# jyakaranda/A-LeGO-LOAM

Measured on AMD Instinct MI355X. Metric: scans/sec (16x1800 LiDAR) full IP->LO->LM loop, higher is better.
Workload: dtype f32/f64

## Files before the change

a-lego-loam_amd/csrc/alego_api.hip:

```cpp
#include <hip/hip_runtime.h>

#include <cmath>
#include <cstdio>
#include <cstdlib>
#include <algorithm>
#include <cstring>
#include <mutex>
#include <string>
#include <vector>

#include "../../include/alego_mi355x.h"
#include "api_gate.h"
#include "dev_common.h"
#include "dev_mem.h"
#include "front_end.h"
#include "lm_ctx.h"
#include "lm_host.h"
#include "merge_math.h"
#include "nn_rules.h"
#include "thin_math.h"
#include "occ_math.h"
#include "loop_ctx.h"
#include "pgraph.h"
#include "prof.h"
// ... 1778 lines not shown
    *count = (int)bytes; *dtype = 3;
    return 0;
  }
  if (s.rfind("rl_", 0) == 0) {
    if (s == "rl_stats") {
      if (cap_bytes < 8) { h->err = "debug_get: buffer too small"; return ALEGO_ERR_CAPACITY; }
      reloc_debug_stats(h->rl, (int*)out);
      *count = 2; *dtype = 2;
      return 0;
    }
    const void* rsrc = nullptr;
    size_t bytes = 0;
    if (reloc_debug_get(h->rl, slot, name, &rsrc, &bytes)) { h->err = std::string("debug_get: ") + name + " needs alego_reloc_enable"; return ALEGO_ERR_ARG; }
    if ((size_t)cap_bytes < bytes) { h->err = "debug_get: buffer too small"; return ALEGO_ERR_CAPACITY; }
    if (bytes) HIP_TRY(h, hipMemcpy(out, rsrc, bytes, hipMemcpyDeviceToHost));
    *count = (int)bytes; *dtype = 3;
    return 0;
  }
  if (s == "fe_cand_span") {
    if (cap_bytes < 8) { h->err = "debug_get: buffer too small"; return ALEGO_ERR_CAPACITY; }
    ((int*)out)[0] = fe_cand_span(d); ((int*)out)[1] = fe_sector_cap(d);
    *count = 2; *dtype = 2;
    return 0;
  }
  if (s == "fe_cand_counts" || s == "fe_cand_lists") {
    if (!fe_fused_eligible(d)) { h->err = "debug_get: " + s + " needs the fused feature extraction"; return ALEGO_ERR_ARG; }
    const bool lists = s == "fe_cand_lists";
    const size_t row = lists ? (size_t)d.P.n_sectors * fe_sector_cap(d) * sizeof(uint2) : (size_t)d.P.n_sectors * 2 * sizeof(int);
    const void* src = lists ? (const void*)st_cand_of(d, slot, 0) : (const void*)st_idx_of(d, slot, 0, F_LFLAT);
    const size_t pitch = lists ? (size_t)((const char*)st_cand_of(d, slot, 1) - (const char*)st_cand_of(d, slot, 0)) : (size_t)((const char*)st_idx_of(d, slot, 1, F_LFLAT) - (const char*)st_idx_of(d, slot, 0, F_LFLAT));
    if ((size_t)cap_bytes < row * d.NS) { h->err = "debug_get: buffer too small"; return ALEGO_ERR_CAPACITY; }
    HIP_TRY(h, hipMemcpy2D(out, row, src, pitch, row, d.NS, hipMemcpyDeviceToHost));
    *count = (int)(row * d.NS / 4); *dtype = 2;
    return 0;
  }
  const size_t base = (size_t)slot * d.N, M = sc[SC_M];
  const size_t fb = fbuf(slot, sc[SC_CUR]);
  int fc[F_KINDS];
  HIP_TRY(h, hipMemcpy(fc, feat_cnt_of(d, fb), sizeof(fc), hipMemcpyDeviceToHost));
  static const char* const cloud[F_KINDS] = {"sharp", "less_sharp", "flat", "less_flat"};
  struct Row { std::string name; const void* row; size_t n; int dtype; };
  std::vector<Row> tab = {
    {"range_img", d.range_img + base, (size_t)d.N, 0}, {"label_img", d.label_img + base, (size_t)d.N, 2}, {"flag_img", d.flag_img + base, (size_t)d.N, 3},
    {"owner", d.owner + base, (size_t)d.N, 2}, {"parent", d.parent + base, (size_t)d.N, 2},
    {"seg_cloud", d.seg_pts + base, M * 4, 0}, {"outlier", d.outlier + base, (size_t)sc[SC_NOUT] * 4, 0},
    {"imu_ptr", imu_ptr_of(d, slot), IMP_N, 2}, {"imu_ring", imu_ring_of(d, slot), imu_ring_n(), 1},
    {"seg_ground", d.seg_ground + base, M, 3}, {"seg_col", d.seg_col + base, M, 2}, {"seg_range", d.seg_range + base, M, 0},
    {"ring_start", ring_start_of(d, slot, 0), (size_t)d.NS, 2}, {"ring_end", ring_end_of(d, slot, 0), (size_t)d.NS, 2},
    {"orientation", ori_of(d, slot), ORI_N, 0}, {"scal", scal_of(d, slot), SC_COUNT, 2},
    {"curv_d", d.cd + base, M, 0}, {"picked_occl", d.picked0 + base, M, 3}, {"point_label", d.plabel + base, M, 2},
    {"lo_surf_corr", lo_corr_of(d, slot, 0), (size_t)fc[F_FLAT] * LC_W, 2}, {"lo_corner_corr", lo_corr_of(d, slot, 1), (size_t)fc[F_SHARP] * LC_W, 2},
    {"lo_state", lo_state_of(d, slot), LO_STATE_N, 1}, {"poses", poses_of(d, slot), PO_W, 1}};
  if (d.P.deskew_mode) tab.push_back({"undistorted", d.seg_dsk + base, (size_t)sc[SC_M_DSK] * 4, 0});
  for (int k = 0; k < F_KINDS; ++k) {
    tab.push_back({cloud[k], feat_of(d, k, fb), (size_t)fc[k] * 4, 0});
    if (k < F_LFLAT) tab.push_back({std::string(cloud[k]) + "_idx", feat_idx_of(d, k, fb), (size_t)fc[k], 2});
  }
  const Row* hit = nullptr;
  for (const Row& r : tab) if (r.name == s) hit = &r;
  if (!hit) return lm_host_debug_get(h->lm, slot, name, out, cap_bytes, count, dtype, &h->err);
  const void* src = hit->row;
  const size_t n = hit->n, esz = hit->dtype == 1 ? 8 : hit->dtype == 3 ? 1 : 4;
  const int dt = hit->dtype;
  if ((size_t)cap_bytes < n * esz) { h->err = "debug_get: buffer too small"; return ALEGO_ERR_CAPACITY; }
  if (n) HIP_TRY(h, hipMemcpy(out, src, n * esz, hipMemcpyDeviceToHost));
  *count = (int)n; *dtype = dt;
  return 0;
}

}
```

a-lego-loam_amd/csrc/kernels_fe2.hip:

```cpp
#include <algorithm>
#include <cstdlib>
#include "dev_common.h"
#include "fe_common.h"
#include "front_end.h"
#include "prof.h"
#include "vgrid.h"

#define FE_MAXH 4096

#ifndef FF_G
#define FF_G 4
#endif
#define FF_LPR (64 / FF_G)
#define FF_HALO 8
#ifndef FC_SPAN
#define FC_SPAN 0
#endif
#ifndef FC_NW
#define FC_NW 4
#endif
#define FF_WIN 256

struct FfLayout {
  int cols, wave_bytes;
// ... 281 lines not shown
    const int ns = R.act0 ? cc[2 * j] : 0, nf = R.act0 ? cc[2 * j + 1] : 0;
    uint2* lst = ff_list(d, slot, rc, j, sector_cap);
    for (int w = gl; w < mw; w += FF_LPR) mk[w] = 0u;
    const int nsw = (int)wave_max_u32((uint32_t)ns), nfw = (int)wave_max_u32((uint32_t)nf);
    constexpr int KU = 32 / FF_LPR;
    if (nsw <= (BIG ? 64 : 32)) ff_pick_regs<(BIG ? 2 : 1) * KU, false>(P, R, ns, lst, 1, mk, mw, gl);
    else if (nsw <= (BIG ? 128 : 64)) ff_pick_regs<(BIG ? 4 : 2) * KU, false>(P, R, ns, lst, 1, mk, mw, gl);
    else if (nsw <= (BIG ? 192 : 96) && !d.opt_fe_cand) ff_pick_regs<(BIG ? 6 : 3) * KU, false>(P, R, ns, lst, 1, mk, mw, gl);
    else ff_pick_mem<false>(P, R, ns, nsw, lst, 1, mk, mw, gl);
    __builtin_amdgcn_wave_barrier();
    if (nfw <= 32 && !(d.opt_fe_cand && nfw > 8)) ff_pick_regs<KU, true>(P, R, nf, lst + sector_cap - 1, -1, mk, mw, gl);
    else if (BIG && nfw <= 64 && !d.opt_fe_cand) ff_pick_regs<2 * KU, true>(P, R, nf, lst + sector_cap - 1, -1, mk, mw, gl);
    else ff_pick_mem<true>(P, R, nf, nfw, lst + sector_cap - 1, -1, mk, mw, gl);
    __builtin_amdgcn_wave_barrier();
  }
  if (rv && gl == 0) {
    int* c = st_cnt_of(d, slot, ring);
    c[F_SHARP] = R.n_sharp; c[F_LSHARP] = R.n_ls; c[F_FLAT] = R.n_flat;
  }
}

#ifndef FO_BLOCK
#define FO_BLOCK 256
#endif
#define FO_NB 256
#define FO_U 4
#define FO_CAP_PCT 72
#define FO_INVALID 0xFFFFFFFFu
#define FO_END 0xFFFFu
#define FO_SPIN_LIMIT (1 << 22)
#define FO_ALIAS_INTS (6 * ((FE_MAXH + LO_CH - 1) / LO_CH) > 768 ? 6 * ((FE_MAXH + LO_CH - 1) / LO_CH) : 768)
#define FO_STATIC_LDS (928 + 4 * FO_ALIAS_INTS)
#ifndef FO_BUDGET_BIG
#define FO_BUDGET_BIG 53248
#endif
#ifndef FO_KEYED
#define FO_KEYED 1
#endif
#ifndef FO_STAGE
#define FO_STAGE 0
#endif
struct FoLayout { int cap; int keyed; };
__host__ __device__ inline FoLayout fo_layout(int H) {
  const int budget = 12 * H + FO_STATIC_LDS > 40960 ? FO_BUDGET_BIG : 40960;
  FoLayout L;
  L.keyed = FO_KEYED && 14 * H + FO_STATIC_LDS <= budget;
  const int by_pct = (H * FO_CAP_PCT / 100 + 15) & ~15, by_lds = (budget - FO_STATIC_LDS - (L.keyed ? 14 : 12) * H) / 16;
  L.cap = !FO_STAGE || by_lds <= 0 ? 0 : (by_pct < by_lds ? by_pct : (by_lds & ~15));
  return L;
}
static size_t fo_lds_bytes(int H) { const FoLayout L = fo_layout(H); return std::max((size_t)(L.keyed ? 14 : 12) * H + (size_t)16 * L.cap, (size_t)6 * 65 * 4); }

DEV_INLINE uint32_t mad_u24(uint32_t a, uint32_t b, uint32_t c) { uint32_t r; asm("v_mad_u32_u24 %0, %1, %2, %3" : "=v"(r) : "v"(a), "v"(b), "v"(c)); return r; }

#ifdef ALEGO_TIMING
__device__ long long fo_times[24];
extern "C" void alego_fo_times(long long* out) { (void)hipMemcpyFromSymbol(out, HIP_SYMBOL(fo_times), sizeof(long long) * 24); }
#ifndef FO_TICK_RING
#define FO_TICK_RING 8
#endif
#define FO_TICK(k) do { if (threadIdx.x == 0 && ring == FO_TICK_RING && blockIdx.x == 0) fo_times[k] = wall_clock64(); } while (0)
#elif defined(FO_STOP_AFTER)
#define FO_TICK(k) do { if ((k) == FO_STOP_AFTER) { if (threadIdx.x == 0) __hip_atomic_store(fe_sync_of(d, slot, ring), (epoch << 16), __ATOMIC_RELAXED, __HIP_MEMORY_SCOPE_AGENT); return; } } while (0)
#else
#define FO_TICK(k)
#endif

DEV_INLINE void fo_picks_out(const DevCtx& d, int slot, unsigned char* smem) {
  fe_concat_picks<FO_BLOCK>(d, slot, fbuf(slot, cur_in_flight(d, slot)), reinterpret_cast<int (*)[65]>(smem), d.n_launch == 1);
}

__global__ void __launch_bounds__(FO_BLOCK) fe_ring_out(DevCtx d) {
  const int slot = blockIdx.x + d.slot0, tid = threadIdx.x, lane = tid & 63;
  const int NS = d.NS, H = d.H;
  extern __shared__ __attribute__((aligned(16))) unsigned char fo_smem[];
  if ((int)blockIdx.x >= d.n_launch) return;
  if ((int)blockIdx.y == NS) { fo_picks_out(d, slot, fo_smem); return; }
  int* scv = scal_of(d, slot);
  __shared__ int s_ticket;
  if (tid == 0) s_ticket = atomicAdd(&scv[SC_FE_TICKET], 1);
  __syncthreads();
  const int ring = min(s_ticket, NS - 1);
  const size_t base = (size_t)slot * d.N;
  const alego_params& P = d.P;
  const int cur = cur_in_flight(d, slot);
  const size_t fb = fbuf(slot, cur);
  const unsigned epoch = (unsigned)scv[SC_FE_EPOCH] & 0xFFFFu;
  const int S = *ring_start_of(d, slot, ring), E = *ring_end_of(d, slot, ring);
  const int n_all = min(max(E - S, 0), H);
  const int n_ls = st_cnt_of(d, slot, ring)[F_LSHARP];
  const int* st_ls = st_idx_of(d, slot, ring, F_LSHARP);
  const float4* seg = d.seg_lo + base;
  float4* s_pt = reinterpret_cast<float4*>(fo_smem);
  const FoLayout lay = fo_layout(H);
  const int cap = lay.cap;
  unsigned char* fv2 = fo_smem + (size_t)16 * cap;
  uint32_t* s_key = reinterpret_cast<uint32_t*>(fv2);
  uint16_t* s_tmp = reinterpret_cast<uint16_t*>(fv2);
  uint32_t* k_tmp = reinterpret_cast<uint32_t*>(fv2);
  uint16_t* s_order = reinterpret_cast<uint16_t*>(fv2 + (lay.keyed ? 12 : 2) * (size_t)H);
  uint32_t* s_rvid = reinterpret_cast<uint32_t*>(fv2 + 4 * (size_t)H);
  uint16_t* s_rstart = reinterpret_cast<uint16_t*>(fv2 + 8 * (size_t)H);
  uint16_t* s_nxt = reinterpret_cast<uint16_t*>(fv2 + 10 * (size_t)H);
  __shared__ uint32_t s_bm[FE_MAXH / 32 + 2];
  constexpr int FO_MAXBOX = (FE_MAXH + LO_CH - 1) / LO_CH;
  constexpr int FO_ALIAS = FO_ALIAS_INTS;
  static_assert(6 * FO_MAXBOX <= FO_ALIAS && 2 * (FO_NB + 1) <= FO_ALIAS && FE_MAXH / 32 + 1 <= FO_ALIAS, "s_alias holds the bucket tables, the hole prefix or the box corners");
  __shared__ int s_alias[FO_ALIAS];
  int* s_boff = s_alias; int* s_bcur = s_alias + FO_NB + 1; int* s_wpre = s_alias;
  uint32_t* s_bx = reinterpret_cast<uint32_t*>(s_alias);
  __shared__ float s_red[6][FO_BLOCK / 64];
  __shared__ int s_scan[FO_BLOCK / 64], s_cntv[FO_BLOCK / 64];
  __shared__ int s_look[3];
  __shared__ int s_rc[64];
  static_assert(FE_MAXH / 64 <= 64 && FO_BLOCK % 64 == 0, "s_rc holds one count per 64 positions of a ring");
  constexpr int NW = FO_BLOCK / 64;
  const int wv = tid >> 6;
  const unsigned long long lt = (1ull << lane) - 1ull;
  if (tid < 64) s_rc[tid] = 0;
  FO_TICK(0);
  float4 keep[FO_U];
#pragma unroll
  for (int u = 0; u < FO_U; ++u) keep[u] = (seg + S)[(unsigned)max(min(tid + u * FO_BLOCK, n_all - 1), 0)];
  const int BW = (n_all + 31) / 32;
  for (int w = tid; w <= BW + 1 && w <= FE_MAXH / 32 + 1; w += FO_BLOCK) s_bm[w] = 0u;
  __syncthreads();
  static_assert(!fe_less_flat_member(1) && !fe_less_flat_member(2) && fe_less_flat_member(0) && fe_less_flat_member(-1), "the labelled holes are exactly the picks of the less_sharp list");
  for (int t = tid; t < n_ls; t += FO_BLOCK) {
    const int i = st_ls[t] - S;
    if (i >= 0 && i < n_all) atomicOr(&s_bm[i >> 5], 1u << (i & 31));
  }
  if (tid < P.n_sectors) {
    int sp, ep;
    fe_sector(P, S, E, tid, sp, ep);
    const int i = sp - S;
    if (fe_sector_lone_point(sp, ep) && i >= 0 && i < n_all) atomicOr(&s_bm[i >> 5], 1u << (i & 31));
  }
  __syncthreads();
  FO_TICK(1);
  auto hole = [&](int i) -> bool { return (s_bm[i >> 5] >> (i & 31)) & 1u; };
  auto prev_kept = [&](int i) -> int {
    uint32_t w = ~s_bm[i >> 5] & (0xFFFFFFFFu >> (31 - (i & 31)));
    int k = i >> 5;
    while (w == 0u && k > 0) { --k; w = ~s_bm[k]; }
    return w ? k * 32 + 31 - __clz((int)w) : -1;
  };
  auto next_kept = [&](int i) -> int {
    const int j = i + 1;
    uint32_t w = ~s_bm[j >> 5] & (0xFFFFFFFFu << (j & 31));
    int k = j >> 5;
    while (w == 0u && k <= BW) { ++k; w = ~s_bm[k]; }
    return w ? k * 32 + __ffs((int)w) - 1 : n_all;
  };
  const float4* seg_ring = seg + S;
#if FO_STAGE
  auto point = [&](int i) -> float4 { if (i < cap) return s_pt[i]; return seg_ring[(unsigned)i]; };
#else
  auto point = [&](int i) -> float4 { return seg_ring[(unsigned)i]; };
#endif
  const float inv = 1.0f / P.less_flat_leaf;
  float mn[3] = {3.402823466e+38f, 3.402823466e+38f, 3.402823466e+38f}, mx[3] = {-3.402823466e+38f, -3.402823466e+38f, -3.402823466e+38f};
  auto wg_box = [&](int nv) -> int {
    nv = wave_sum_i32(nv);
#pragma unroll
    for (int a = 0; a < 3; ++a) { mn[a] = wave_min_f32(mn[a]); mx[a] = wave_max_f32(mx[a]); }
    __syncthreads();
    if (lane == 0) {
      s_cntv[wv] = nv;
#pragma unroll
      for (int a = 0; a < 3; ++a) { s_red[a][wv] = mn[a]; s_red[3 + a][wv] = mx[a]; }
    }
    __syncthreads();
    nv = 0;
#pragma unroll
    for (int w = 0; w < NW; ++w) nv += s_cntv[w];
#pragma unroll
    for (int a = 0; a < 3; ++a) {
      mn[a] = s_red[a][0]; mx[a] = s_red[3 + a][0];
#pragma unroll
      for (int w = 1; w < NW; ++w) { mn[a] = fminf(mn[a], s_red[a][w]); mx[a] = fmaxf(mx[a], s_red[3 + a][w]); }
    }
    return nv;
  };
  auto bbox_exact = [&]() {
#pragma unroll
    for (int a = 0; a < 3; ++a) { mn[a] = 3.402823466e+38f; mx[a] = -3.402823466e+38f; }
#pragma nounroll
    for (int i = tid; i < n_all; i += FO_BLOCK) {
      if (hole(i)) continue;
      vgr_box_add(mn, mx, point(i));
    }
    (void)wg_box(0);
  };
  int nval = 0;
  {
    int nh = 0;
    for (int w = tid; w <= BW; w += FO_BLOCK) nh += __popc(s_bm[w]);
    for (int i0 = tid; i0 < n_all; i0 += FO_BLOCK * FO_U) {
      float4 pt[FO_U];
#pragma unroll
      for (int u = 0; u < FO_U; ++u) pt[u] = i0 == tid ? keep[u] : seg_ring[(unsigned)min(i0 + u * FO_BLOCK, n_all - 1)];
#pragma unroll
      for (int u = 0; u < FO_U; ++u) {
#if FO_STAGE
        const int i = i0 + u * FO_BLOCK;
        if (i < min(n_all, cap)) s_pt[i] = pt[u];
#endif
        vgr_box_add(mn, mx, pt[u]);
      }
    }
    nval = n_all - wg_box(nh);
  }
  FO_TICK(2);
  bool passthrough = false;
  if (nval > 0 && vgr_leaf_too_small(mn, mx, inv)) { bbox_exact(); passthrough = vgr_leaf_too_small(mn, mx, inv); }
  int nout = 0, nrv = 0, nruns = 0, vex = 0;
  if (passthrough) {
    if (tid == 0) { int acc = 0; for (int w = 0; w <= BW; ++w) { s_wpre[w] = acc; acc += __popc(s_bm[w]); } }
    nout = nval;
  } else if (nval > 0) {
    const VgrGeom g = vgr_geom(mn, mx, inv);
    const bool u24 = (unsigned)g.divb[0] < (1u << 24) && (unsigned)g.divb[1] < (1u << 24) && (unsigned)g.divb[2] < (1u << 24) && g.mul2 < (1u << 24);
    auto key_chunk = [&](int c, float4 own) {
      const int i = c * FO_BLOCK + tid;
      uint32_t key = FO_INVALID;
      if (i < n_all) {
        const int src = prev_kept(i);
        float4 q = own;
        if (src != i) q = point(max(src, 0));
        int i0, i1, i2;
        vgr_coords(g, q, inv, &i0, &i1, &i2);
        const uint32_t id = u24 ? mad_u24((uint32_t)i2, g.mul2, mad_u24((uint32_t)i1, g.mul1, (uint32_t)i0)) : (uint32_t)i0 + (uint32_t)i1 * g.mul1 + (uint32_t)i2 * g.mul2;
        key = src < 0 ? FO_INVALID : id;
        s_key[i] = key;
      }
      const uint32_t prev = (uint32_t)__builtin_amdgcn_update_dpp((int)key, (int)key, 0x138, 0xF, 0xF, false);
      const unsigned long long m = __ballot(i < n_all && key != prev);
      if (lane == 0) s_rc[c * NW + wv] = (int)__popcll(m);
    };
#pragma unroll
    for (int c = 0; c < FO_U; ++c) if (c * FO_BLOCK < n_all) key_chunk(c, keep[c]);
#pragma nounroll
    for (int c = FO_U; c * FO_BLOCK < n_all; ++c) key_chunk(c, seg_ring[(unsigned)min(c * FO_BLOCK + tid, n_all - 1)]);
    __syncthreads();
    {
      const int p0 = lane * 64;
      const int ex = wave_excl_scan(s_rc[lane] + ((p0 < n_all && (p0 == 0 || s_key[p0] != s_key[p0 - 1])) ? 1 : 0), &nruns);
#pragma nounroll
      for (int c = 0; c * FO_BLOCK < n_all; ++c) {
        const int i = c * FO_BLOCK + tid;
        const uint32_t mykey = i < n_all ? s_key[i] : 0u;
        const bool head = i < n_all && (i == 0 || mykey != s_key[i - 1]);
        const unsigned long long m = __ballot(head);
        const int r0 = __builtin_amdgcn_readlane(ex, __builtin_amdgcn_readfirstlane(c * NW + wv));
        if (head) {
          const int r = r0 + (int)__popcll(m & lt);
          s_rvid[r] = mykey;
          s_rstart[r] = (uint16_t)i;
        }
        if (i < n_all) {
          const int j = next_kept(i);
          s_nxt[i] = (uint16_t)((j < n_all && s_key[min(j, n_all - 1)] == mykey) ? j : FO_END);
        }
      }
    }
    __syncthreads();
    FO_TICK(3);
    {
      const FeBuckets bk = fe_buckets(g.T, FO_NB);
      const int shift = bk.shift, nb = bk.nb;
      fe_buckets_clear<FO_BLOCK>(nb, s_boff);
      __syncthreads();
      FO_TICK(9);
      for (int r = tid; r < nruns; r += FO_BLOCK) { const uint32_t v = s_rvid[r]; if (v != FO_INVALID) atomicAdd(&s_boff[fe_bucket_of(bk, v) + 1], 1); }
      __syncthreads();
      FO_TICK(10);
      fe_buckets_scan<FO_BLOCK, FO_NB>(nb, s_boff, s_bcur, s_scan);
      __syncthreads();
      nrv = s_boff[nb];
      FO_TICK(11);
      const bool keyed = lay.keyed && shift <= 20;
      const uint32_t lowmask = (1u << shift) - 1u;
      for (int r = tid; r < nruns; r += FO_BLOCK) {
        const uint32_t v = s_rvid[r];
        if (v != FO_INVALID) {
          const int pos = atomicAdd(&s_bcur[fe_bucket_of(bk, v)], 1);
          if (keyed) k_tmp[pos] = ((v & lowmask) << 12) | (uint32_t)r;
          else s_tmp[pos] = (uint16_t)r;
        }
      }
      __syncthreads();
      FO_TICK(12);
#ifdef ALEGO_TIMING
      if (tid == 0 && ring == FO_TICK_RING && blockIdx.x == 0) { int mxb = 0; for (int b = 0; b < nb; ++b) mxb = max(mxb, s_boff[b + 1] - s_boff[b]); fo_times[16] = n_all; fo_times[17] = nruns; fo_times[18] = nrv; fo_times[19] = nb; fo_times[20] = mxb; }
#endif
      for (int t = tid; t < nrv; t += FO_BLOCK) {
        const uint32_t mine = keyed ? k_tmp[t] : 0u;
        const int r = keyed ? (int)(mine & 0xFFFu) : (int)s_tmp[t];
        const uint32_t v = s_rvid[r];
        const int b = fe_bucket_of(bk, v);
        const int bs = s_boff[b], be = s_boff[b + 1];
        int rank = bs;
        if (keyed) {
#pragma nounroll
          for (int q = bs; q < be; ++q) rank += k_tmp[q] < mine ? 1 : 0;
        } else {
#pragma nounroll
          for (int q = bs; q < be; ++q) { const int o = s_tmp[q]; const uint32_t u = s_rvid[o]; rank += (u < v) || (u == v && o < r); }
        }
        s_order[rank] = (uint16_t)r;
      }
    }
    if (tid < 64) s_rc[tid] = 0;
    __syncthreads();
    FO_TICK(4);
// ... 149 lines not shown
```

a-lego-loam_amd/csrc/kernels_lm.hip:

```cpp
#include <cstddef>
#include <cstring>

#include "../../include/alego_mi355x.h"
#include "dev_cost.h"
#include "nn_rules.h"
#include "remap_math.h"
#include "prof.h"
#include "kf_store.h"
#include "gmap.h"
#include "vgrid.h"
#include "vox_merge.h"

#define LM_BLOCK 256

DEV_INLINE double* ldp(const LmCtx& L, int slot) { return L.ld + (size_t)slot * LD_COUNT; }
DEV_INLINE int* lip(const LmCtx& L, int slot) { return L.li + (size_t)slot * LI_COUNT; }

DEV_INLINE void lm_map_update(const LmCtx& L, int slot, int* li, int merge) {
  const int nkf = li[LI_NKF];
  if (nkf == 0) return;
  int* rec = L.rec + (size_t)slot * L.K;
  const int cnt = li[LI_REC_CNT];
  bool changed = false;
  if (cnt < L.K) {
// ... 151 lines not shown
  __shared__ int s_base[LT_T];
  __shared__ float s_red[6][LT_T / 64];
  __shared__ int s_w[LT_T / 64];
  int state = 0;
  if (li[LI_RUN]) {
    const float FMAX = 3.402823466e+38f;
    int no = li[LI_NCUR_O];
    const int nin = min(li[LI_NIN_O], L.in_cap_o);
    if (nin <= LT_OCAP) {
      const float4* in = L.in_outl + (size_t)slot * L.in_cap_o;
      float4* out = L.cur_outl_ds + (size_t)slot * L.kf_cap_o;
      const int cap = L.kf_cap_o;
      const float inv = 1.0f / d.P.lm_leaf_outlier;
      int nvox = 0, full = nin;
      if (nin > 0) {
        float mn[3] = {FMAX, FMAX, FMAX}, mx[3] = {-FMAX, -FMAX, -FMAX};
        for (int i = tid; i < nin; i += LT_T) vgr_box_add(mn, mx, in[i]);
        lt_box_reduce(mn, mx, s_red);
        if (vgr_leaf_too_small(mn, mx, inv)) {
          for (int i = tid; i < min(nin, cap); i += LT_T) out[i] = in[i];
        } else {
          const VgrGeom g = vgr_geom(mn, mx, inv);
          for (int i = tid; i < nin; i += LT_T) s_key[i] = vgr_id(g, in[i], inv);
          lt_order(s_key, s_skey, s_idx, nin);
          for (int t0 = 0; t0 < nin; t0 += LT_T) {
            const int m = t0 + tid;
            const bool head = m < nin && (m == 0 || s_skey[m] != s_skey[m - 1]);
            int tot;
            const int r = nvox + block_excl_scan<LT_T / 64>(head ? 1 : 0, s_w, &tot);
            if (head && r < cap) {
              int b = m + 1;
              while (b < nin && s_skey[b] == s_skey[m]) ++b;
              out[r] = vm_centroid([&](int j) { return in[s_idx[j]]; }, m, b);
            }
            nvox += tot;
          }
          full = nvox;
        }
      }
      no = min(full, cap);
      if (tid == 0) { li[LI_NCUR_O] = no; if (full > cap) li[LI_OVERFLOW] = 1; }
      __syncthreads();
    }
    const int ns = li[LI_NCUR_S];
    if (ns + no > L.total_cap) { no = L.total_cap - ns; if (tid == 0) li[LI_OVERFLOW] = 1; }
    const int n = ns + no, cap = L.total_cap;
    const float4* S = L.cur_surf_ds + (size_t)slot * L.kf_cap_s;
    const float4* O = L.cur_outl_ds + (size_t)slot * L.kf_cap_o;
    float4* out = L.cur_total_ds + (size_t)slot * L.total_cap;
    const float inv = 1.0f / d.P.lm_leaf_surf;
    const int c = (ns + LT_T - 1) / LT_T, c0 = min(ns, tid * c), c1 = min(ns, c0 + c);
    bool refuse = no > LT_OCAP;
    int heads = 0;
    if (!refuse && n > 0) {
      float mn[3] = {FMAX, FMAX, FMAX}, mx[3] = {-FMAX, -FMAX, -FMAX};
      int good = 1;
      for (int j = tid; j < no; j += LT_T) { const float4 p = O[j]; vgr_box_add(mn, mx, p); good &= vm_finite(p); s_key[j] = vkey_of(p, inv); s_osb[j] = -1; }
      lt_order(s_key, s_skey, s_idx, no);
      vm_u64 kprev = 0;
      int ole_prev = 0;
      if (c0 > 0 && c0 < c1) { kprev = vkey_of(S[c0 - 1], inv); ole_prev = vm_count_le(s_skey, no, kprev); }
      for (int b0 = c0; b0 < c1; b0 += LT_B) {
        float4 p[LT_B];
#pragma unroll
        for (int k = 0; k < LT_B; ++k) p[k] = S[min(b0 + k, c1 - 1)];
#pragma unroll
        for (int k = 0; k < LT_B; ++k) {
          const int i = b0 + k;
          if (i < c1) {
            vgr_box_add(mn, mx, p[k]);
            const vm_u64 key = vkey_of(p[k], inv);
            good &= vm_finite(p[k]) && (i == 0 || kprev <= key);
            const int ol = vm_count_less(s_skey, no, key);
            for (int j = ole_prev; j < ol; ++j) s_osb[j] = tid << 16 | heads;
            heads += (i == 0 || kprev != key) ? 1 : 0;
            kprev = key; ole_prev = vm_count_le(s_skey, no, key);
          }
        }
      }
      if ((c0 < c1 && c1 == ns) || (ns == 0 && tid == 0)) for (int j = ole_prev; j < no; ++j) s_osb[j] = tid << 16 | heads;
      lt_box_reduce(mn, mx, s_red);
      good = __syncthreads_and(good);
      refuse = vm_refuse(good != 0, no, mn, mx, inv);
    }
    if (!refuse) {
      int nsh;
      const int base = block_excl_scan<LT_T / 64>(heads, s_w, &nsh);
      s_base[tid] = base;
      int noo = 0;
      for (int t0 = 0; t0 < no; t0 += LT_T) {
        const int j = t0 + tid;
        const bool oh = j < no && s_osb[j] >= 0 && (j == 0 || s_skey[j - 1] != s_skey[j]);
        int tot;
        const int e = noo + block_excl_scan<LT_T / 64>(oh ? 1 : 0, s_w, &tot);
        if (j < no) s_oop[j] = e;
        noo += tot;
      }
      if (tid == 0) s_oop[no] = noo;
      __syncthreads();
      vm_u64 kprev = c0 > 0 && c0 < c1 ? vkey_of(S[c0 - 1], inv) : 0;
      int hl = 0;
      for (int b0 = c0; b0 < c1; b0 += LT_B) {
        float4 p[LT_B + 1];
#pragma unroll
        for (int k = 0; k <= LT_B; ++k) p[k] = S[min(b0 + k, ns - 1)];
#pragma unroll
        for (int k = 0; k < LT_B; ++k) {
          const int i = b0 + k;
          if (i < c1) {
            const vm_u64 key = vkey_of(p[k], inv);
            if (i == 0 || kprev != key) {
              const int ol = vm_count_less(s_skey, no, key), ole = vm_count_le(s_skey, no, key);
              const int r = base + hl + s_oop[ol];
              ++hl;
              if (r < cap) {
                int nsr = 1;
                if (i + 1 < ns && vkey_of(p[k + 1], inv) == key) while (i + nsr < ns && vkey_of(S[i + nsr], inv) == key) ++nsr;
                out[r] = vm_centroid([&](int q) { return q == 0 ? p[k] : (q < nsr ? S[i + q] : O[s_idx[ol + q - nsr]]); }, 0, nsr + ole - ol);
              }
            }
            kprev = key;
          }
        }
      }
      for (int j = tid; j < no; j += LT_T) {
        if (s_osb[j] >= 0 && (j == 0 || s_skey[j - 1] != s_skey[j])) {
          const int r = s_base[s_osb[j] >> 16] + (s_osb[j] & 0xFFFF) + s_oop[j];
          if (r < cap) {
            int e = j + 1;
            while (e < no && s_skey[e] == s_skey[j]) ++e;
            out[r] = vm_centroid([&](int q) { return O[s_idx[q]]; }, j, e);
          }
        }
      }
      const int nvox = nsh + noo;
      if (tid == 0) { li[LI_NTOTAL] = n; li[LI_NTOTAL_DS] = min(nvox, cap); if (nvox > cap) li[LI_OVERFLOW] = 1; li[LI_TM_FAST] += 1; }
    } else {
      float4* t = L.cur_total + (size_t)slot * L.total_cap;
      for (int i = tid; i < ns; i += LT_T) t[i] = S[i];
      for (int i = tid; i < no; i += LT_T) t[ns + i] = O[i];
      if (tid == 0) { li[LI_NTOTAL] = n; li[LI_TM_LIST] += 1; }
      state = n > W.small_max ? 2 : 1;
    }
  }
  if (tid == 0) {
    if (state == 1) W.list_small[atomicAdd(&W.cnt[0], 1)] = slot - L.vox_slot0;
    else if (state == 2) W.list_big[atomicAdd(&W.cnt[1], 1)] = slot - L.vox_slot0;
    if (blockIdx.x == 0) { W.cnt_next[0] = 0; W.cnt_next[1] = 0; }
  }
}

DEV_INLINE int grid_cell(const GridGeom& g, float x, float y, float z, int* cx, int* cy, int* cz) {
  *cx = nn_lm_coord(x, g.inv) - g.ox; *cy = nn_lm_coord(y, g.inv) - g.oy; *cz = nn_lm_coord(z, g.inv) - g.oz;
  return nn_lm_index(*cx, *cy, *cz, g.gx, g.gy, g.gz);
}

__global__ void __launch_bounds__(LM_BLOCK) lm_grid_build(DevCtx d, LmCtx L) {
  const int slot = blockIdx.y + d.slot0, m = blockIdx.x;
  const int* li = lip(L, slot);
  if (!li[LI_REBUILD]) return;
  __shared__ GridGeom s_g;
  __shared__ int s[LM_BLOCK / 64];
  __shared__ int s_run;
  if (threadIdx.x == 0) {
    const unsigned* bb = d.opt_map_merge ? L.map_bbox + ((size_t)slot * 2 + m) * 8 : L.vox_bbox + ((size_t)(slot - L.vox_slot0) * 2 + m) * 8;
// ... 1023 lines not shown
```

a-lego-loam_amd/csrc/kernels_lo.hip:

```cpp
#include <algorithm>
#include <cstdlib>
#include <type_traits>
#include "dev_cost.h"
#include "front_end.h"
#include "lm_ctx.h"
#include "nn_rules.h"
#include "prof.h"

#define LO_BLOCK 256
#ifndef LO_SOLVE_BLOCK
#define LO_SOLVE_BLOCK 64
#endif

DEV_INLINE void pose_rotation(const double* p, double R[9]) {
  const DQuat q = dq_zyx(p[5], p[4], p[3]);
  dq_to_mat(q, R);
}
DEV_INLINE void store_pose_rotation(double* st) {
  double R[9];
  pose_rotation(st + LS_PARAMS, R);
#pragma unroll
  for (int k = 0; k < 9; ++k) st[LS_ROT + k] = R[k];
#pragma unroll
  for (int k = 0; k < 6; ++k) st[LS_ROT_P + k] = st[LS_PARAMS + k];
// ... 298 lines not shown
        int cb[LO_NB];
        pop_boxes(surv, c0, cb);
        best = nn_eval(cb, best);
      }
    }
    bj = group_min_u64<16>(best);
    }
    LA_TICK(4);
    const bool found = nn_lo_found(nn_key_d2(bj), nfd);
    if (found) closest = nn_key_index(bj);
    const int cref = found ? closest : 0;
    const int cr = (int)tg[cref].w;
    const int W = d.P.ring_window;
    const int rlo = nn_walk_ring(cr, -W, d.NS), rhi = nn_walk_ring(cr, W, d.NS), crc = nn_walk_ring(cr, 0, d.NS);
    const int lo = found ? s_roff[rlo] : 0, hi = found ? s_roff[rhi + 1] : 0;
    const int same_lo = s_roff[crc], same_hi = s_roff[crc + 1];
    WalkBest b2{nfd, 0x7fffffff, -1}, b3{nfd, 0x7fffffff, -1};
    auto walk_one = [&](int k, bool valid, const float4& a) {
      if (!valid || k < lo || k >= hi || k == closest) return;
      const double pd = nn_walk_d2(a.x - sx, a.y - sy, a.z - sz);
      if (!(pd < nfd)) return;
      const int rank = nn_walk_rank(k, closest, hi);
      const bool same = k >= same_lo && k < same_hi;
      const bool w2 = nn_walk_second(kind, same) && nn_walk_better(pd, rank, b2.dist, b2.rank);
      const bool w3 = nn_walk_third(kind, same) && nn_walk_better(pd, rank, b3.dist, b3.rank);
      b2.dist = w2 ? pd : b2.dist; b2.rank = w2 ? rank : b2.rank; b2.idx = w2 ? k : b2.idx;
      b3.dist = w3 ? pd : b3.dist; b3.rank = w3 ? rank : b3.rank; b3.idx = w3 ? k : b3.idx;
    };
    auto walk_eval = [&](const int (&cb)[LO_NB]) {
      int k[TPL * LO_NB], bs[LO_NB], bl[LO_NB];
      bool v[TPL * LO_NB];
      float4 a[TPL * LO_NB];
#pragma unroll
      for (int u = 0; u < LO_NB; ++u) box_span(cb[u], bs[u], bl[u]);
#pragma unroll
      for (int u = 0; u < TPL * LO_NB; ++u) { k[u] = bs[u / TPL] + l16 + 16 * (u % TPL); v[u] = l16 + 16 * (u % TPL) < bl[u / TPL]; }
#pragma unroll
      for (int u = 0; u < TPL * LO_NB; ++u) a[u] = tg[v[u] ? k[u] : 0];
#pragma unroll
      for (int u = 0; u < TPL * LO_NB; ++u) walk_one(k[u], v[u], a[u]);
    };
    const int cw0 = found ? s_boff[rlo] : 0, cw1 = found ? s_boff[rhi + 1] - 1 : -1;
    const int same_b0 = s_boff[crc], same_b1 = s_boff[crc + 1];
    auto box_class = [&](int c, bool& inS, bool& inO) {
      const bool own = c >= same_b0 && c < same_b1;
      inS = kind == 0 && own;
      inO = !own;
    };
    auto lb_f64 = [&](int c) -> double {
      float dx, dy, dz;
      box_diff(c, dx, dy, dz);
      return nn_walk_d2(dx, dy, dz);
    };
    unsigned long long mo = ~0ull;
    for (int it = 0; __ballot(cw0 + it * 16 <= cw1); ++it) {
      const int c = cw0 + it * 16 + l16;
      if (c <= cw1) {
        bool inS, inO;
        box_class(c, inS, inO);
        if (inO) {
          const unsigned long long k = ((unsigned long long)__double_as_longlong(lb_f64(c)) & 0xFFFFFFFF00000000ull) | (uint32_t)c;
          mo = k < mo ? k : mo;
        }
      }
    }
    mo = group_min_u64<16>(mo);
    LA_TICK(5);
    const int cseedS = cw1 >= cw0 ? min(max(same_b0 + (closest - same_lo) / LO_CH, cw0), cw1) : -1, cseedO = mo == ~0ull ? -1 : (int)(uint32_t)mo;
    { int cb[LO_NB]; for (int u = 0; u < LO_NB; ++u) cb[u] = -1; cb[0] = cseedS; cb[1] = cseedO != cseedS ? cseedO : -1; walk_eval(cb); }
    const double seenS = b2.dist, seenO3 = b3.dist;
    double inS = nfd, inO = seenS;
    if (kind == 0) { inS = seenS; inO = seenO3; }
    const double boundS = __longlong_as_double((long long)group_min_u64<16>((unsigned long long)__double_as_longlong(inS)));
    LA_TICK(6);
    const double boundO = __longlong_as_double((long long)group_min_u64<16>((unsigned long long)__double_as_longlong(inO)));
    if (lane == 0) LA_COUNT(0, 1);
    if (l16 == 0) LA_COUNT(3, max(cw1 - cw0 + 1, 0));
    for (int it0 = 0; __ballot(cw0 + it0 * 16 <= cw1); it0 += 4) {
      const int cbase = cw0 + it0 * 16;
      unsigned long long surv = 0ull;
#pragma unroll
      for (int g = 0; g < 4; ++g) {
        const int c = cbase + g * 16 + l16;
        if (!__ballot(c <= cw1)) break;
        bool take = false;
        if (c <= cw1 && c != cseedS && c != cseedO) {
          bool inS, inO;
          box_class(c, inS, inO);
          const double lb = lb_f64(c);
          take = (inS && lb <= boundS) || (inO && lb <= boundO);
        }
        surv |= (unsigned long long)row_bits(__ballot(take), lane) << (16 * g);
      }
      if (l16 == 0) LA_COUNT(2, __popcll(surv));
      while (__ballot(surv != 0ull)) {
        if (lane == 0) LA_COUNT(1, 1);
        int cb[LO_NB];
#pragma unroll
        for (int u = 0; u < LO_NB; ++u) { cb[u] = surv ? cbase + __ffsll((long long)surv) - 1 : -1; surv &= surv - 1ull; }
        walk_eval(cb);
      }
    }
    LA_TICK(7);
    b2 = walk_reduce_row(b2);
    idx2 = b2.idx;
    if (kind == 0) { b3 = walk_reduce_row(b3); idx3 = b3.idx; }
  }
  LA_TICK(8);
  if (l16 == 0 && store) {
    int* row = lo_corr_of(d, slot, kind, q);
    const bool ok = nn_lo_row_ok(kind, idx2, idx3);
    row[0] = q; row[1] = ok ? closest : -1; row[2] = idx2; row[3] = idx3;
  }
  }
}

template <int kind, int BOXCAP = LO_BOX_LDS>
__global__ void __launch_bounds__(LO_BLOCK) lo_assoc(DevCtx d, int box_lds_max) {
  lo_assoc_body<kind, LO_BLOCK, BOXCAP>(d, box_lds_max, blockIdx.x + d.slot0, blockIdx.y, gridDim.y);
}

struct LoRowPts { float4 c, a, b, m; };
DEV_INLINE LoRowPts lo_row_points(const float4* qpts, const float4* tg, const int4& r, int kind, bool ok) {
  return LoRowPts{qpts[ok ? r.x : 0], tg[ok ? r.y : 0], tg[ok ? r.z : 0], tg[(ok && kind == 0) ? r.w : 0]};
}
template <int kind, bool FULL, bool GENERIC>
DEV_INLINE void lo_eval_row(const double cp[3], const double a[3], const double b[3], const double c[3], const PoseTerms& T, double huber, double acc[28]) {
  if constexpr (FULL) {
    double res, J[6];
    eval_block(kind == 0 ? BLK_SURF : BLK_CORNER, cp, a, b, c, 0.0, T, &res, J);
    if constexpr (GENERIC) accumulate_block(res, J, huber, acc);
    else accumulate_block_cols<kind == 0 ? COLS_SURF : COLS_CORNER>(res, J, huber, acc);
  } else accumulate_cost(eval_block_residual<kind == 0 ? BLK_SURF : BLK_CORNER>(cp, a, b, c, 0.0, T), huber, acc[27]);
}
template <int BLK, int kind, bool FULL = true, bool GENERIC = true>
DEV_INLINE void lo_eval_rows(const DevCtx& d, int slot, int n, const PoseTerms& T, double acc[28]) {
  const float4* qpts = feat_of(d, kind == 0 ? F_FLAT : F_SHARP, fidx_cur(d, slot));
  const float4* tg = feat_of(d, kind == 0 ? F_LFLAT : F_LSHARP, fidx_last(d, slot));
  const int* rows = lo_corr_of(d, slot, kind);
  for (int i = threadIdx.x; i < n; i += BLK) {
    const int4 r = *reinterpret_cast<const int4*>(rows + (size_t)i * LC_W);
    if (r.y < 0) continue;
    const LoRowPts p = lo_row_points(qpts, tg, r, kind, true);
// ... 399 lines not shown
```

a-lego-loam_amd/csrc/vox_merge.h:

```cpp
#ifndef ALEGO_VOX_MERGE_H_
#define ALEGO_VOX_MERGE_H_
#include "vgrid.h"

#define LT_OCAP 512

typedef unsigned long long vm_u64;

VGR_FN bool vm_finite(const float4& p) { return fabsf(p.x) <= 3.402823466e+38f && fabsf(p.y) <= 3.402823466e+38f && fabsf(p.z) <= 3.402823466e+38f; }

VGR_FN int vm_rank(const vm_u64* key, int n, int i) {
  const vm_u64 k = key[i];
  int r = 0;
  for (int j = 0; j < n; ++j) r += (key[j] < k || (key[j] == k && j < i)) ? 1 : 0;
  return r;
}

VGR_FN int vm_count_less(const vm_u64* sorted, int n, vm_u64 key) {
  int lo = 0, hi = n;
  while (lo < hi) { const int mid = (lo + hi) >> 1; if (sorted[mid] < key) lo = mid + 1; else hi = mid; }
  return lo;
}
VGR_FN int vm_count_le(const vm_u64* sorted, int n, vm_u64 key) {
  int lo = 0, hi = n;
  while (lo < hi) { const int mid = (lo + hi) >> 1; if (sorted[mid] <= key) lo = mid + 1; else hi = mid; }
  return lo;
}

VGR_FN bool vm_refuse(bool sound, int no, const float mn[3], const float mx[3], float inv) {
  if (!sound || no > LT_OCAP) return true;
  if (!vkey_holds_box(mn, mx, inv) || vgr_leaf_too_small(mn, mx, inv)) return true;
  return vgr_geom(mn, mx, inv).T > 0xFFFFFFFFull;
}

template <class At>
VGR_FN float4 vm_centroid(At at, int a, int b) {
  float sx = 0.f, sy = 0.f, sz = 0.f, si = 0.f;
  for (int j = a; j < b; ++j) { const float4 p = at(j); sx += p.x; sy += p.y; sz += p.z; si += p.w; }
  const float fn = (float)(b - a);
  float4 c;
  c.x = sx / fn; c.y = sy / fn; c.z = sz / fn; c.w = si / fn;
  return c;
}

#endif
```

Baseline: 498,700.

## Pair keys per thread in feature output, narrow merge searches, reuse LO bounds

The feature-output kernel now assigns two adjacent points per thread. That lets it skip the voxel-id computation for holes, write keys with vector stores, and build run heads and next links in pairs. The local-map merge kernel replaces full binary searches with searches started from the previous bound and runs them only at key changes. The LO walk keeps the first groups' lower bounds in registers and skips boxes outside both classes. A debug table also gains extra rows. Together these cut redundant arithmetic and LDS traffic, but add register pressure and complexity in the pairing logic.

```diff
diff --git a/a-lego-loam_amd/csrc/alego_api.hip b/a-lego-loam_amd/csrc/alego_api.hip
--- a/a-lego-loam_amd/csrc/alego_api.hip
+++ b/a-lego-loam_amd/csrc/alego_api.hip
@@ -1854,6 +1854,15 @@
     {"lo_surf_corr", lo_corr_of(d, slot, 0), (size_t)fc[F_FLAT] * LC_W, 2}, {"lo_corner_corr", lo_corr_of(d, slot, 1), (size_t)fc[F_SHARP] * LC_W, 2},
     {"lo_state", lo_state_of(d, slot), LO_STATE_N, 1}, {"poses", poses_of(d, slot), PO_W, 1}};
   if (d.P.deskew_mode) tab.push_back({"undistorted", d.seg_dsk + base, (size_t)sc[SC_M_DSK] * 4, 0});
+  {
+    int nbox = 0;
+    HIP_TRY(h, hipMemcpy(&nbox, ring_boff_of(d, fb, RO_LFLAT) + d.NS, sizeof(int), hipMemcpyDeviceToHost));
+    nbox = std::min(std::max(nbox, 0), d.lo_box_cap);
+    tab.push_back({"less_flat_ring_off", ring_off_of(d, fb, RO_LFLAT), (size_t)d.NS + 1, 2});
+    tab.push_back({"less_flat_ring_boff", ring_boff_of(d, fb, RO_LFLAT), (size_t)d.NS + 1, 2});
+    tab.push_back({"less_flat_boxes", lo_box_of(d, lo_row(fb, box_set_of(F_LFLAT))), (size_t)nbox * 8, 0});
+    tab.push_back({"fe_ring_counts", st_cnt_of(d, slot, 0), (size_t)d.NS * ST_W, 2});
+  }
   for (int k = 0; k < F_KINDS; ++k) {
     tab.push_back({cloud[k], feat_of(d, k, fb), (size_t)fc[k] * 4, 0});
     if (k < F_LFLAT) tab.push_back({std::string(cloud[k]) + "_idx", feat_idx_of(d, k, fb), (size_t)fc[k], 2});
diff --git a/a-lego-loam_amd/csrc/kernels_fe2.hip b/a-lego-loam_amd/csrc/kernels_fe2.hip
--- a/a-lego-loam_amd/csrc/kernels_fe2.hip
+++ b/a-lego-loam_amd/csrc/kernels_fe2.hip
@@ -357,6 +357,8 @@
 static size_t fo_lds_bytes(int H) { const FoLayout L = fo_layout(H); return std::max((size_t)(L.keyed ? 14 : 12) * H + (size_t)16 * L.cap, (size_t)6 * 65 * 4); }
 
 DEV_INLINE uint32_t mad_u24(uint32_t a, uint32_t b, uint32_t c) { uint32_t r; asm("v_mad_u32_u24 %0, %1, %2, %3" : "=v"(r) : "v"(a), "v"(b), "v"(c)); return r; }
+static_assert(FO_U % 2 == 0, "keep[] holds whole pairs");
+DEV_INLINE int fo_keep_pos(int tid, int u) { return (u >> 1) * 2 * FO_BLOCK + 2 * tid + (u & 1); }
 
 #ifdef ALEGO_TIMING
 __device__ long long fo_times[24];
@@ -426,7 +428,7 @@
   FO_TICK(0);
   float4 keep[FO_U];
 #pragma unroll
-  for (int u = 0; u < FO_U; ++u) keep[u] = (seg + S)[(unsigned)max(min(tid + u * FO_BLOCK, n_all - 1), 0)];
+  for (int u = 0; u < FO_U; ++u) keep[u] = (seg + S)[(unsigned)max(min(fo_keep_pos(tid, u), n_all - 1), 0)];
   const int BW = (n_all + 31) / 32;
   for (int w = tid; w <= BW + 1 && w <= FE_MAXH / 32 + 1; w += FO_BLOCK) s_bm[w] = 0u;
   __syncthreads();
@@ -508,7 +510,7 @@
 #pragma unroll
       for (int u = 0; u < FO_U; ++u) {
 #if FO_STAGE
-        const int i = i0 + u * FO_BLOCK;
+        const int i = i0 == tid ? fo_keep_pos(tid, u) : i0 + u * FO_BLOCK;
         if (i < min(n_all, cap)) s_pt[i] = pt[u];
 #endif
         vgr_box_add(mn, mx, pt[u]);
@@ -526,46 +528,65 @@
   } else if (nval > 0) {
     const VgrGeom g = vgr_geom(mn, mx, inv);
     const bool u24 = (unsigned)g.divb[0] < (1u << 24) && (unsigned)g.divb[1] < (1u << 24) && (unsigned)g.divb[2] < (1u << 24) && g.mul2 < (1u << 24);
-    auto key_chunk = [&](int c, float4 own) {
-      const int i = c * FO_BLOCK + tid;
-      uint32_t key = FO_INVALID;
-      if (i < n_all) {
-        const int src = prev_kept(i);
-        float4 q = own;
-        if (src != i) q = point(max(src, 0));
-        int i0, i1, i2;
-        vgr_coords(g, q, inv, &i0, &i1, &i2);
-        const uint32_t id = u24 ? mad_u24((uint32_t)i2, g.mul2, mad_u24((uint32_t)i1, g.mul1, (uint32_t)i0)) : (uint32_t)i0 + (uint32_t)i1 * g.mul1 + (uint32_t)i2 * g.mul2;
-        key = src < 0 ? FO_INVALID : id;
-        s_key[i] = key;
-      }
-      const uint32_t prev = (uint32_t)__builtin_amdgcn_update_dpp((int)key, (int)key, 0x138, 0xF, 0xF, false);
-      const unsigned long long m = __ballot(i < n_all && key != prev);
-      if (lane == 0) s_rc[c * NW + wv] = (int)__popcll(m);
+    constexpr int FO_PAIR = 2 * FO_BLOCK;
+    auto voxel_id = [&](float4 q) -> uint32_t {
+      int i0, i1, i2;
+      vgr_coords(g, q, inv, &i0, &i1, &i2);
+      return u24 ? mad_u24((uint32_t)i2, g.mul2, mad_u24((uint32_t)i1, g.mul1, (uint32_t)i0)) : (uint32_t)i0 + (uint32_t)i1 * g.mul1 + (uint32_t)i2 * g.mul2;
     };
-#pragma unroll
-    for (int c = 0; c < FO_U; ++c) if (c * FO_BLOCK < n_all) key_chunk(c, keep[c]);
+    auto key_chunk = [&](int c, float4 own_a, float4 own_b) {
+      const int ia = c * FO_PAIR + 2 * tid, ib = ia + 1;
+      uint32_t key_a = FO_INVALID, key_b = FO_INVALID;
+      if (ia < n_all) {
+        const uint32_t hb = s_bm[ia >> 5] >> (ia & 31);
+        int src = ia;
+        float4 q = own_a;
+        if (hb & 1u) { src = prev_kept(ia); q = point(max(src, 0)); }
+        const uint32_t id = voxel_id(q);
+        key_a = src < 0 ? FO_INVALID : id;
+        if (ib < n_all) {
+          key_b = key_a;
+          if (!(hb & 2u)) key_b = voxel_id(own_b);
+          *reinterpret_cast<uint2*>(s_key + ia) = make_uint2(key_a, key_b);
+        } else {
+          s_key[ia] = key_a;
+        }
+      }
+      const uint32_t prev = (uint32_t)__builtin_amdgcn_update_dpp((int)key_a, (int)key_b, 0x138, 0xF, 0xF, false);
+      const unsigned long long ma = __ballot(ia < n_all && key_a != prev), mb = __ballot(ib < n_all && key_b != key_a);
+      if (lane == 0) s_rc[c * NW + wv] = (int)__popcll(ma) + (int)__popcll(mb);
+    };
+#pragma unroll
+    for (int c = 0; c < FO_U / 2; ++c) if (c * FO_PAIR < n_all) key_chunk(c, keep[2 * c], keep[2 * c + 1]);
 #pragma nounroll
-    for (int c = FO_U; c * FO_BLOCK < n_all; ++c) key_chunk(c, seg_ring[(unsigned)min(c * FO_BLOCK + tid, n_all - 1)]);
+    for (int c = FO_U / 2; c * FO_PAIR < n_all; ++c) {
+      const int ia = c * FO_PAIR + 2 * tid;
+      key_chunk(c, seg_ring[(unsigned)min(ia, n_all - 1)], seg_ring[(unsigned)min(ia + 1, n_all - 1)]);
+    }
     __syncthreads();
     {
-      const int p0 = lane * 64;
+      const int p0 = lane * 128;
       const int ex = wave_excl_scan(s_rc[lane] + ((p0 < n_all && (p0 == 0 || s_key[p0] != s_key[p0 - 1])) ? 1 : 0), &nruns);
 #pragma nounroll
-      for (int c = 0; c * FO_BLOCK < n_all; ++c) {
-        const int i = c * FO_BLOCK + tid;
-        const uint32_t mykey = i < n_all ? s_key[i] : 0u;
-        const bool head = i < n_all && (i == 0 || mykey != s_key[i - 1]);
-        const unsigned long long m = __ballot(head);
+      for (int c = 0; c * FO_PAIR < n_all; ++c) {
+        const int ia = c * FO_PAIR + 2 * tid, ib = ia + 1;
+        const bool in_a = ia < n_all, in_b = ib < n_all;
+        uint32_t key_a = 0u, key_b = 0u;
+        if (in_b) { const uint2 kk = *reinterpret_cast<const uint2*>(s_key + ia); key_a = kk.x; key_b = kk.y; }
+        else if (in_a) key_a = s_key[ia];
+        const bool head_a = in_a && (ia == 0 || key_a != s_key[max(ia - 1, 0)]), head_b = in_b && key_b != key_a;
+        const unsigned long long ma = __ballot(head_a), mb = __ballot(head_b);
         const int r0 = __builtin_amdgcn_readlane(ex, __builtin_amdgcn_readfirstlane(c * NW + wv));
-        if (head) {
-          const int r = r0 + (int)__popcll(m & lt);
-          s_rvid[r] = mykey;
-          s_rstart[r] = (uint16_t)i;
-        }
-        if (i < n_all) {
-          const int j = next_kept(i);
-          s_nxt[i] = (uint16_t)((j < n_all && s_key[min(j, n_all - 1)] == mykey) ? j : FO_END);
+        const int ra = r0 + (int)__popcll(ma & lt) + (int)__popcll(mb & lt);
+        if (head_a) { s_rvid[ra] = key_a; s_rstart[ra] = (uint16_t)ia; }
+        if (head_b) { const int rb = ra + (head_a ? 1 : 0); s_rvid[rb] = key_b; s_rstart[rb] = (uint16_t)ib; }
+        if (in_b) {
+          const int j = next_kept(ib);
+          const uint16_t nb = (uint16_t)((j < n_all && s_key[min(j, n_all - 1)] == key_b) ? j : FO_END);
+          s_nxt[ia] = hole(ib) ? nb : (uint16_t)(key_b == key_a ? ib : FO_END);
+          s_nxt[ib] = nb;
+        } else if (in_a) {
+          s_nxt[ia] = (uint16_t)FO_END;
         }
       }
     }
diff --git a/a-lego-loam_amd/csrc/kernels_lm.hip b/a-lego-loam_amd/csrc/kernels_lm.hip
--- a/a-lego-loam_amd/csrc/kernels_lm.hip
+++ b/a-lego-loam_amd/csrc/kernels_lm.hip
@@ -227,6 +227,7 @@
     const int c = (ns + LT_T - 1) / LT_T, c0 = min(ns, tid * c), c1 = min(ns, c0 + c);
     bool refuse = no > LT_OCAP;
     int heads = 0;
+    int o_lo = 0, o_hi = 0;
     if (!refuse && n > 0) {
       float mn[3] = {FMAX, FMAX, FMAX}, mx[3] = {-FMAX, -FMAX, -FMAX};
       int good = 1;
@@ -235,6 +236,7 @@
       vm_u64 kprev = 0;
       int ole_prev = 0;
       if (c0 > 0 && c0 < c1) { kprev = vkey_of(S[c0 - 1], inv); ole_prev = vm_count_le(s_skey, no, kprev); }
+      o_lo = ole_prev;
       for (int b0 = c0; b0 < c1; b0 += LT_B) {
         float4 p[LT_B];
 #pragma unroll
@@ -246,13 +248,18 @@
             vgr_box_add(mn, mx, p[k]);
             const vm_u64 key = vkey_of(p[k], inv);
             good &= vm_finite(p[k]) && (i == 0 || kprev <= key);
-            const int ol = vm_count_less(s_skey, no, key);
-            for (int j = ole_prev; j < ol; ++j) s_osb[j] = tid << 16 | heads;
-            heads += (i == 0 || kprev != key) ? 1 : 0;
-            kprev = key; ole_prev = vm_count_le(s_skey, no, key);
+            if (i == 0 || kprev != key) {
+              const int ol = vm_count_less_from(s_skey, no, key, ole_prev);
+              for (int j = ole_prev; j < ol; ++j) s_osb[j] = tid << 16 | heads;
+              heads += 1;
+              ole_prev = vm_count_le_from(s_skey, no, key, ol);
+              if (i == c0) o_lo = ol;
+            }
+            kprev = key;
           }
         }
       }
+      o_hi = ole_prev;
       if ((c0 < c1 && c1 == ns) || (ns == 0 && tid == 0)) for (int j = ole_prev; j < no; ++j) s_osb[j] = tid << 16 | heads;
       lt_box_reduce(mn, mx, s_red);
       good = __syncthreads_and(good);
@@ -275,6 +282,8 @@
       __syncthreads();
       vm_u64 kprev = c0 > 0 && c0 < c1 ? vkey_of(S[c0 - 1], inv) : 0;
       int hl = 0;
+      const bool osearch = o_hi != o_lo;
+      int obound = o_lo;
       for (int b0 = c0; b0 < c1; b0 += LT_B) {
         float4 p[LT_B + 1];
 #pragma unroll
@@ -285,7 +294,8 @@
           if (i < c1) {
             const vm_u64 key = vkey_of(p[k], inv);
             if (i == 0 || kprev != key) {
-              const int ol = vm_count_less(s_skey, no, key), ole = vm_count_le(s_skey, no, key);
+              int ol = obound, ole = obound;
+              if (osearch) { ol = vm_count_less_from(s_skey, no, key, obound); ole = vm_count_le_from(s_skey, no, key, ol); obound = ole; }
               const int r = base + hl + s_oop[ol];
               ++hl;
               if (r < cap) {
diff --git a/a-lego-loam_amd/csrc/kernels_lo.hip b/a-lego-loam_amd/csrc/kernels_lo.hip
--- a/a-lego-loam_amd/csrc/kernels_lo.hip
+++ b/a-lego-loam_amd/csrc/kernels_lo.hip
@@ -374,8 +374,27 @@
       box_diff(c, dx, dy, dz);
       return nn_walk_d2(dx, dy, dz);
     };
+    constexpr int LA_KEEP = kind == 0 ? 4 : 1;
     unsigned long long mo = ~0ull;
-    for (int it = 0; __ballot(cw0 + it * 16 <= cw1); ++it) {
+    double lbk[LA_KEEP];
+#pragma unroll
+    for (int it = 0; it < LA_KEEP; ++it) {
+      lbk[it] = 0.0;
+      const int c = cw0 + it * 16 + l16;
+      if (c <= cw1) {
+        bool inS, inO;
+        box_class(c, inS, inO);
+        if (inS || inO) {
+          const double lb = lb_f64(c);
+          lbk[it] = lb;
+          if (inO) {
+            const unsigned long long k = ((unsigned long long)__double_as_longlong(lb) & 0xFFFFFFFF00000000ull) | (uint32_t)c;
+            mo = k < mo ? k : mo;
+          }
+        }
+      }
+    }
+    for (int it = LA_KEEP; __ballot(cw0 + it * 16 <= cw1); ++it) {
       const int c = cw0 + it * 16 + l16;
       if (c <= cw1) {
         bool inS, inO;
@@ -401,6 +420,7 @@
     for (int it0 = 0; __ballot(cw0 + it0 * 16 <= cw1); it0 += 4) {
       const int cbase = cw0 + it0 * 16;
       unsigned long long surv = 0ull;
+      static_assert(LA_KEEP <= 4, "the kept bounds are groups of the first turn");
 #pragma unroll
       for (int g = 0; g < 4; ++g) {
         const int c = cbase + g * 16 + l16;
@@ -409,8 +429,10 @@
         if (c <= cw1 && c != cseedS && c != cseedO) {
           bool inS, inO;
           box_class(c, inS, inO);
-          const double lb = lb_f64(c);
-          take = (inS && lb <= boundS) || (inO && lb <= boundO);
+          if (inS || inO) {
+            const double lb = it0 == 0 && g < LA_KEEP ? lbk[g < LA_KEEP ? g : 0] : lb_f64(c);
+            take = (inS && lb <= boundS) || (inO && lb <= boundO);
+          }
         }
         surv |= (unsigned long long)row_bits(__ballot(take), lane) << (16 * g);
       }
diff --git a/a-lego-loam_amd/csrc/vox_merge.h b/a-lego-loam_amd/csrc/vox_merge.h
--- a/a-lego-loam_amd/csrc/vox_merge.h
+++ b/a-lego-loam_amd/csrc/vox_merge.h
@@ -25,6 +25,20 @@
   while (lo < hi) { const int mid = (lo + hi) >> 1; if (sorted[mid] <= key) lo = mid + 1; else hi = mid; }
   return lo;
 }
+VGR_FN int vm_count_less_from(const vm_u64* sorted, int n, vm_u64 key, int lo) {
+  if (lo >= n || !(sorted[lo] < key)) return lo;
+  int hi = n;
+  ++lo;
+  while (lo < hi) { const int mid = (lo + hi) >> 1; if (sorted[mid] < key) lo = mid + 1; else hi = mid; }
+  return lo;
+}
+VGR_FN int vm_count_le_from(const vm_u64* sorted, int n, vm_u64 key, int lo) {
+  if (lo >= n || !(sorted[lo] <= key)) return lo;
+  int hi = n;
+  ++lo;
+  while (lo < hi) { const int mid = (lo + hi) >> 1; if (sorted[mid] <= key) lo = mid + 1; else hi = mid; }
+  return lo;
+}
 
 VGR_FN bool vm_refuse(bool sound, int no, const float mn[3], const float mx[3], float inv) {
   if (!sound || no > LT_OCAP) return true;
```

Result: no change. 502,700 (median of 6 runs) (+0.8%).
